# patngnw/NewsRecommendation

Measured on AMD Instinct MI355X. Metric: train impressions/sec @ batch 512, NRMS, higher is better.
Workload: dtype bf16; 1 GPU; NRMS train step (fwd+bwd+Adam), MIND-small shapes: title_len=30, history=50, npratio=4, 300-d word table; per_gpu_batch=512, global_batch=512, vocab_rows=30000, freeze_embedding=False, compact_history=False, dense_batch=False, feed=resident, deterministic=False, optimizer=flat bucket + HIP fused Adam, parallelism=dp1

## Files before the change

include/nrhip.h:

```cpp
#ifndef NRHIP_H
#define NRHIP_H

#include <stddef.h>
#include <stdint.h>

#ifdef __cplusplus
extern "C" {
#endif

#define NR_F32 0
#define NR_BF16 1

#define NR_OK 0
#define NR_ERR_ARG 1
#define NR_ERR_HIP 2

#define NR_SRC_DENSE 0
#define NR_SRC_GATHER 1

typedef void* nr_stream_t;

int nr_version(void);
int nr_last_error(char* buf, size_t n);
int nr_abi_sizes(size_t* out, int n);
// ... 111 lines not shown
                     int dtype, nr_stream_t stream);

typedef struct {
  int M, K, N, dtype;
  int src_kind;
  const void* x;
  int ldx;
  const int32_t* ids;
  int ids_stride;
  const void* w;
  int ldw;
  const float* bias;
  const void* w_t;
  int ldwt;
  size_t dout_ws_bytes;
  int table_rows;
} nr_linear_desc;
size_t nr_linear_workspace_bytes(const nr_linear_desc* d);
int nr_linear_fwd(const nr_linear_desc* d, float* out, int ld_out, nr_stream_t stream);
int nr_linear_bwd(const nr_linear_desc* d, const float* dout, int ld_dout, void* dout_ws, float* dw,
                  float* db, float* dtable, nr_stream_t stream);

int nr_score_ce_fwd(const float* cand, int ld_cand, const float* user, const int64_t* label, float* score,
                    float* loss, float* lossvec, int B, int C, int N, nr_stream_t stream);
int nr_score_ce_bwd(const float* cand, int ld_cand, const float* user, const int64_t* label,
                    const float* score, const float* gloss, const float* gscore, float* dcand, int ld_dcand,
                    float* duser, int B, int C, int N, nr_stream_t stream);
int nr_score_eval(const float* news_vecs, int ld_news, const int32_t* cand_ids, const int32_t* imp_of,
                  const float* user, int ld_user, float* score, int n_cand, int N, nr_stream_t stream);

int nr_assemble_batch(const int32_t* news_combined, int n_rows, int F, const int32_t* hist_idx, const int32_t* pos_idx,
                      const int32_t* neg_idx, const int64_t* label, int B, int H, int K, int32_t* history, int32_t* candidate,
                      int32_t* bad, nr_stream_t stream);

int nr_stack_rows(const int32_t* a, int rows_a, const int32_t* b, int rows_b, int F, const float* mask_b, int32_t* out,
                  int32_t* flags, nr_stream_t stream);

size_t nr_eval_metrics_workspace_bytes(int n_imp);
int nr_eval_metrics(const float* score, const int32_t* label, const int32_t* offsets, int n_imp, int max_cand, double* per_imp,
                    size_t per_imp_bytes, double* sums, nr_stream_t stream);

int nr_adam_step(float* param, float* grad, float* exp_avg, float* exp_avg_sq, size_t n, float lr, float beta1, float beta2, float eps,
                 int step, float grad_scale, int zero_grad, nr_stream_t stream);
#define NR_ADAM_PACK_MAX 4
typedef struct {
  size_t first, count;
  int cols, ld_dst;
// ... 22 lines not shown
```

newsrecommendation_amd/_lib.py:

```python
from __future__ import annotations

import ctypes as C
import os
import subprocess
import threading

NR_F32, NR_BF16 = 0, 1
NR_SRC_DENSE, NR_SRC_GATHER = 0, 1

_HERE = os.path.dirname(os.path.abspath(__file__))
LIB_PATH = os.environ.get("NRHIP_LIB") or os.path.join(_HERE, "libnrhip.so")
CSRC_DIR = os.path.join(_HERE, "csrc")

c_f32p = C.POINTER(C.c_float)
c_i32p = C.POINTER(C.c_int32)
c_i64p = C.POINTER(C.c_int64)


class MhsaDesc(C.Structure):
    _fields_ = [("n", C.c_int), ("L", C.c_int), ("d_model", C.c_int), ("heads", C.c_int), ("d_head", C.c_int),
                ("dtype", C.c_int), ("src_kind", C.c_int), ("x", C.c_void_p), ("ldx", C.c_int), ("ids", C.c_void_p),
                ("p_in", C.c_float), ("seed_in", C.c_uint32), ("p_out", C.c_float), ("seed_out", C.c_uint32),
                ("mask", C.c_void_p), ("w_qkv", C.c_void_p), ("ldw", C.c_int), ("b_qkv", C.c_void_p),
                ("x_rows", C.c_void_p), ("ld_rows", C.c_int), ("row_ws", C.c_void_p), ("row_ws_bytes", C.c_size_t),
# ... 61 lines not shown
    "nr_adam_step": [_vp, _vp, _vp, _vp, C.c_size_t, _f, _f, _f, _f, _i, _f, _i, _vp],
    "nr_adam_step_packed": [_vp, _vp, _vp, _vp, C.c_size_t, _f, _f, _f, _f, _i, _f, _i, _vp, _i, _vp],
    "nr_check_ids": [_vp, _i, _i, _i, _vp, _vp],
    "nr_check_labels": [_vp, _i, _i, _vp, _vp],
    "nr_cast_pad": [_vp, _i, _i, _i, _vp, _i, _i, _i, _vp],
    "nr_cast_pad_batch": [_vp, _i, _i, _vp],
    "nr_pack_conv_w": [_vp, _i, _i, _vp, _i, _i, _vp],
    "nr_unpack_conv_dw": [_vp, _i, _i, _i, _vp, _i, _vp],
    "nr_embed_gather_fwd": [_vp, _i, _i, _vp, _i, _i, _i, _vp, _i, _vp],
    "nr_embed_gather_bwd": [_vp, _i, _vp, _i, _i, _i, _vp, _i, _vp],
    "nr_gather_cast_fwd": [_vp, _i, _vp, _i, _i, _vp, _i, _i, _vp],
    "nr_mhsa_fwd_fused": [C.POINTER(MhsaDesc)],
    "nr_mhsa_compact_rows": [C.POINTER(MhsaDesc)],
    "nr_mhsa_fwd": [C.POINTER(MhsaDesc), _vp, _vp, _vp],
    "nr_mhsa_bwd": [C.POINTER(MhsaDesc), _vp, _vp, _vp, _vp, _i, _vp, _vp, _vp, _vp, _vp],
    "nr_conv1d_k3_fwd": [C.POINTER(ConvDesc), _vp, _vp],
    "nr_conv1d_k3_bwd": [C.POINTER(ConvDesc), _vp, _vp, _vp, _vp],
    "nr_additive_pool_fwd": [C.POINTER(PoolDesc), _vp, _vp, _vp, _i, _vp],
    "nr_additive_pool_bwd": [C.POINTER(PoolDesc), _vp, _vp, _vp, _i, _vp, _i, _vp, _vp, _vp, _vp, _vp, _vp, _vp, _vp],
    "nr_pad_blend_fwd": [_vp, _vp, _vp, _vp, _i, _i, _i, _i, _vp],
    "nr_pad_blend_bwd": [_vp, _vp, _vp, _vp, _i, _i, _i, _i, _vp],
    "nr_linear_fwd": [C.POINTER(LinearDesc), _vp, _i, _vp],
    "nr_linear_bwd": [C.POINTER(LinearDesc), _vp, _i, _vp, _vp, _vp, _vp, _vp],
    "nr_score_ce_fwd": [_vp, _i, _vp, _vp, _vp, _vp, _vp, _i, _i, _i, _vp],
    "nr_score_ce_bwd": [_vp, _i, _vp, _vp, _vp, _vp, _vp, _vp, _i, _vp, _i, _i, _i, _vp],
    "nr_score_eval": [_vp, _i, _vp, _vp, _vp, _i, _vp, _i, _i, _vp],
    "nr_gemm_nt": [_i, _vp, _i, _vp, _i, _vp, _i, _vp, _i, _i, _i, _i, _i, _vp],
    "nr_gemm_tn": [_i, _vp, _i, _vp, _i, _vp, _i, _vp, _i, _i, _i, _vp],
    "nr_dropout_mask": [_vp, _u32, _f, _u32, _vp],
    "nr_prof_enable": [_i],
    "nr_prof_collect": [C.c_char_p, C.c_size_t],
    "nr_prof_filter": [C.c_char_p],
    "nr_debug_nt_trace": [_vp, _i],
}

_lib = None
_lock = threading.Lock()


def build(force: bool = False) -> str:
    if force or not os.path.exists(LIB_PATH):
        subprocess.run(["make", "-C", CSRC_DIR, "-j4"], check=True)
    elif _stale():
        subprocess.run(["make", "-C", CSRC_DIR, "-j4"], check=True)
    return LIB_PATH


# ... 74 lines not shown
```

newsrecommendation_amd/csrc/nr_api.hip:

```cpp
#include <stdarg.h>
#include <stdio.h>
#include <stdlib.h>
#include <string.h>

#include "nr_gemm.h"

int nr_launch_attn(bool bwd, int dtype, const void* qkv, const float* mask, void* y, const void* dy, void* dqkv, int n, int L,
                   int heads, int d_head, const DropCfg& drop, hipStream_t stream, const uint32_t* tmask = nullptr,
                   const float* bias = nullptr, const int32_t* seq_list = nullptr, const int32_t* seq_count = nullptr,
                   const int32_t* needed = nullptr);
bool nr_attn_pad_ok(int dtype, int L, int d_head, const void* p0, const void* p1);
bool nr_attn_rowsub_ok(int dtype, int L, int d_head, int heads);
bool nr_attn_compact_ok(int dtype, int L, int d_head, int heads);
int nr_launch_attn_bwd_compact(const void* qkv, const float* mask, const void* dy, void* dqkv, int n, int L, int heads, int d_head,
                               const DropCfg& drop, hipStream_t stream, const uint32_t* tmask, const float* bias, const int32_t* seq_list,
                               const int32_t* seq_count, const int32_t* pos, void* dump, float* db, const int32_t* nzf);
int nr_launch_attn_gather_fwd(const void* proj_table, const int32_t* ids, const float* mask, void* y, int n, int L, int heads,
                              int d_head, const DropCfg& drop, hipStream_t stream);
int nr_launch_pool_core_fwd(int dtype, const void* x, const void* e, const float* w2, const float* b2, const float* mask,
                            float* alpha, float* out, int ld_out, int n, int L, int N, int q, hipStream_t s,
                            const int32_t* needed = nullptr);
int nr_launch_pool_core_bwd(int dtype, const void* x, const void* e, const float* w2, const float* alpha, const float* g,
                            int ld_g, void* dpre, float* partial, float* dw2, float* db2, int n, int L, int N, int q,
                            hipStream_t s, const int32_t* seq_nz = nullptr);
// ... 224 lines not shown
  memset(&e, 0, sizeof(e));
  e.C = C; e.ldc = ldc; e.out_dtype = out_dtype; e.bias = bias; e.act_tanh = act_tanh;
  e.drop = nr_make_drop(0.f, 0);
  return e;
}

static int mhsa_rows(const nr_mhsa_desc* d, RowSrc* out) {
  RowSrc s = dense_rows(d->x, d->ldx, d->d_model);
  if (d->src_kind == NR_SRC_GATHER) {
    NR_CHECK_ARG(d->ids != nullptr, "mhsa: gather source without ids");
    s.kind = ROWS_GATHER;
    s.ids = d->ids;
  } else {
    NR_CHECK_ARG(d->src_kind == NR_SRC_DENSE, "mhsa: bad src_kind %d", d->src_kind);
  }
  s.drop = nr_make_drop(d->p_in, d->seed_in);
  *out = s;
  return NR_OK;
}

struct MhsaWs {
  size_t live_idx, live_ids, dead_idx, tmask, slab, seq, sort_idx, sort_ids, hist, cursor, pos, sort_k, dump, tn_scratch, tn_floats, total;
};
static MhsaWs mhsa_ws_layout(int n, int L, int table_rows, int N3 = 0, int Kp = 0) {
  const size_t M = (size_t)n * L;
  MhsaWs w;
  w.live_idx = 4; w.live_ids = 4 + M; w.dead_idx = 4 + 2 * M; w.tmask = 4 + 3 * M;
  w.slab = w.tmask + n;
  w.seq = w.slab + n + 4 + M / 32 + 4;
  w.sort_idx = (w.seq + 4 + n + 4 + 3) / 4 * 4;
  w.sort_ids = w.sort_idx + (table_rows > 0 ? (M + 3) / 4 * 4 : 0);
  w.hist = w.sort_ids + (table_rows > 0 ? (M + 3) / 4 * 4 : 0);
  w.cursor = w.hist + (table_rows > 0 ? (size_t)table_rows + 8 : 0);
  w.pos = (w.cursor + (table_rows > 0 ? (size_t)table_rows + 8 : 0) + 3) / 4 * 4;
  w.sort_k = w.pos + (table_rows > 0 ? (M + 3) / 4 * 4 : 0);
  w.dump = w.sort_k + (table_rows > 0 ? (M + 3) / 4 * 4 : 0);
  w.tn_scratch = (w.dump + (table_rows > 0 ? 1024 : 0) + 3) / 4 * 4;
  w.tn_floats = (table_rows > 0 && N3 >= 8 && Kp >= 8 && M % 32 == 0) ? nr_gemm_tn_scratch_floats((int)M, N3, Kp) : 0;
  w.total = w.tn_scratch + w.tn_floats;
  return w;
}
static MhsaWs mhsa_ws_of(const nr_mhsa_desc* d) {
  const bool gather = d->src_kind == NR_SRC_GATHER;
  const int ch = dtype_ok(d->dtype) ? nr_chunk(d->dtype) : 4;
  return mhsa_ws_layout(d->n, d->L, gather ? d->table_rows : 0, gather && d->dtype == NR_BF16 ? 3 * d->heads * d->d_head : 0,
                        gather && d->dtype == NR_BF16 ? round_up(d->d_model, ch) : 0);
}
static size_t conv_ws_elems(int n, int T) { return (size_t)n + 4 + ((size_t)n * T) / 32 + 12; }
int nr_pool_partial_rows(int n);
static size_t pool_ws_used(int n, int q) { return ((size_t)nr_pool_partial_rows(n) * (q + 1) + 3) / 4 * 4; }
static size_t pool_ws_ints(int n, int L, int q) { return (pool_ws_used(n, q) + (size_t)n + 8 + ((size_t)n * L) / 32 + 4 + 3) / 4 * 4; }
static size_t pool_tn_floats(int n, int L, int q, int N, int dtype) {
  const size_t M = (size_t)n * L;
  return (dtype == NR_BF16 && q >= 8 && N >= 8 && M % 32 == 0 && M > 0) ? nr_gemm_tn_scratch_floats((int)M, q, N) : 0;
}
static size_t pool_ws_elems(int n, int L, int q, int N = 0, int dtype = NR_F32) { return pool_ws_ints(n, L, q) + pool_tn_floats(n, L, q, N, dtype); }

static bool pool_has_flags(const nr_pool_desc* d) {
  const int M = d->n * d->L;
  return !nr_opt(NR_OPT_NO_SLABS) && d->dtype == NR_BF16 && M % 32 == 0 && d->L <= 32 && nr_gemm_tn_slabs_ok(d->q, d->N, M, d->q, d->N);
}

static bool conv_slab_shape(const nr_conv_desc* d) {
  const int M = d->n * d->T;
  return !nr_opt(NR_OPT_NO_SLABS) && d->dtype == NR_BF16 && d->x_rows != nullptr && M % 32 == 0 && d->T <= 32 && d->N % 8 == 0 &&
         nr_gemm_tn_slabs_ok(d->N, d->ld_rows, M, d->N, 3 * d->Dp);
}

static bool mhsa_compact_rows(const nr_mhsa_desc* d) {
// ... 424 lines not shown
        if (d->table_rows > 0 && !nr_opt(NR_OPT_NO_SCATTER_SORT)) {
          if ((rc = nr_launch_sort_rows_by_id(d->row_ws, ep.row_idx, ep.row_ids, M, d->table_rows, d->row_ws + W.hist,
                                              d->row_ws + W.sort_idx, d->row_ws + W.sort_ids, s)))
            return rc;
          ep.row_idx = d->row_ws + W.sort_idx; ep.row_ids = d->row_ws + W.sort_ids;
        }
      }
      rc = nr_launch_gemm_nt(d->dtype, G, w_qkv_t, ldwt, M, d->d_model, 3 * N, EPI_SCATTER, ep, s);
    } else {
      NR_CHECK_ARG(dx != nullptr && dtable == nullptr, "mhsa_bwd: dense source takes dx, not dtable");
      NR_CHECK_ARG(d->p_in == 0.f, "mhsa_bwd: input dropout on a dense source is not supported");
      NR_CHECK_ARG(d->d_model % 4 == 0, "mhsa_bwd: d_model=%d must be a multiple of 4", d->d_model);
      EpiArgs ep = store_epi(dx, d->ldx, d->dtype, nullptr, 0);
      rc = nr_launch_gemm_nt(d->dtype, G, w_qkv_t, ldwt, M, d->d_model, 3 * N, EPI_STORE, ep, s);
    }
  }
  if (rc) return rc;
  if (ph_dw) {
    if (slab_ws != nullptr) {
      if ((rc = nr_launch_gemm_tn_slabs(dqkv, 3 * N, d->x_rows, d->ld_rows, dw_qkv, d->d_model, db_qkv, M, 3 * N, Kp, 3 * N, d->d_model,
                                        slab_ws + d->n + 4, slab_ws + d->n, s, 0,
                                        W.tn_floats ? reinterpret_cast<float*>(d->row_ws + W.tn_scratch) : nullptr, W.tn_floats)))
        return rc;
    } else if ((rc = nr_launch_gemm_tn(d->dtype, dqkv, 3 * N, Xs, dw_qkv, d->d_model, db_qkv, M, 3 * N, Kp, 3 * N, d->d_model, s))) {
      return rc;
    }
  }
  if (fork) {
    const int rj = side_join(s);
    if (rc == NR_OK) rc = rj;
  }
  const int rd = det.end();
  return rc ? rc : rd;
}

static int conv_rows(const nr_conv_desc* d, RowSrc* out) {
  NR_CHECK_ARG(d != nullptr, "conv1d: null descriptor");
  NR_CHECK_ARG(dtype_ok(d->dtype), "conv1d: bad dtype %d", d->dtype);
  const int ch = nr_chunk(d->dtype);
  NR_CHECK_ARG(d->n >= 0 && d->T >= 1 && d->D >= 1 && d->N >= 1 && d->Dp >= d->D && d->Dp % ch == 0,
               "conv1d: bad shape n=%d T=%d D=%d Dp=%d N=%d", d->n, d->T, d->D, d->Dp, d->N);
  NR_CHECK_ARG(d->N % ch == 0, "conv1d: N=%d must be a multiple of %d", d->N, ch);
  NR_CHECK_ARG(d->n == 0 || (d->table && d->ids && d->w_pack && d->bias && d->ids_stride >= 1), "conv1d: null operand");
  NR_CHECK_ARG((uint64_t)d->n * d->T * (uint64_t)d->D < 0xffffffffull, "conv1d: problem too large for 32-bit element counters");
  RowSrc s = dense_rows(d->table, d->Dp, d->D);
  s.kind = ROWS_IM2COL3;
  s.ids = d->ids; s.ids_stride = d->ids_stride; s.Tlen = d->T;
// ... 120 lines not shown
  const int32_t* zero_flags = ws != nullptr ? ws : d->seq_needed;
  if (ws != nullptr && dx != nullptr && w1_t != nullptr && !det.on() && nr_pool_fused_bwd_ok(d->dtype, d->n, d->L, d->N, d->q, ldw1t) && ld_g % 4 == 0 &&
      ((((uintptr_t)d->x) | ((uintptr_t)e) | ((uintptr_t)w1_t) | ((uintptr_t)dpre) | ((uintptr_t)dx) | ((uintptr_t)g)) & 15) == 0 && d->N % 8 == 0) {
    int rows = 0;
    if ((rc = nr_launch_pool_fused_bwd(d->x, d->N, e, d->q, alpha, g, ld_g, d->w2, w1_t, ldw1t, dpre, d->q, dx, d->N, partial,
                                       nr_pool_partial_rows(d->n), ws, d->n, d->L, d->N, d->q, s, &rows, d->dx_far_unwritten)))
      return rc;
    if ((rc = nr_launch_colsum_split(partial, rows, d->q + 1, d->q + 1, dw2, d->q, db2, s))) return rc;
    if ((rc = nr_launch_live_slabs(ws, d->n, d->L, s))) return rc;
    return nr_launch_gemm_tn_slabs(dpre, d->q, d->x, d->N, dw1, d->N, db1, M, d->q, d->N, d->q, d->N, ws + d->n + 4, ws + d->n, s, 0,
                                   tn_floats ? tn_scratch : nullptr, tn_floats);
  }
  if ((rc = nr_launch_pool_core_bwd(d->dtype, d->x, e, d->w2, alpha, g, ld_g, dpre, partial, dw2, db2, d->n, d->L, d->N, d->q, s, zero_flags)))
    return rc;
  RowSrc X = dense_rows(d->x, d->N, d->N);
  const bool fork = dx != nullptr && side_enabled() && M >= 65536 && !det.on();
  hipStream_t s2 = s;
  if (fork && (rc = side_fork(s, &s2))) return rc;
  if (ws != nullptr) {
    if ((rc = nr_launch_live_slabs(ws, d->n, d->L, s))) return rc;
    if ((rc = nr_launch_gemm_tn_slabs(dpre, d->q, d->x, d->N, dw1, d->N, db1, M, d->q, d->N, d->q, d->N, ws + d->n + 4, ws + d->n, s, 0,
                                      tn_floats ? tn_scratch : nullptr, tn_floats)))
      return rc;
  } else if ((rc = nr_launch_gemm_tn(d->dtype, dpre, d->q, X, dw1, d->N, db1, M, d->q, d->N, d->q, d->N, s))) {
    return rc;
  }
  if (dx != nullptr) {
    NR_CHECK_ARG(w1_t != nullptr && ldw1t >= d->q, "additive_pool_bwd: w1_t [N, >=q] needed for dx");
    RowSrc P = dense_rows(dpre, d->q, d->q);
    EpiArgs ep = store_epi(dx, d->N, d->dtype, nullptr, 0);
    ep.rowscale = alpha; ep.G = g; ep.ldg = ld_g; ep.L = d->L;
    ep.seq_nz = zero_flags;
    rc = nr_launch_gemm_nt(d->dtype, P, w1_t, ldw1t, M, d->N, d->q, EPI_POOLBWD, ep, s2);
  }
  if (fork) {
    const int rj = side_join(s);
    if (rc == NR_OK) rc = rj;
  }
  return rc;
}

static int linear_rows(const nr_linear_desc* d, RowSrc* out) {
  NR_CHECK_ARG(d != nullptr, "linear: null descriptor");
  NR_CHECK_ARG(dtype_ok(d->dtype), "linear: bad dtype %d", d->dtype);
  const int ch = nr_chunk(d->dtype);
  NR_CHECK_ARG(d->M >= 0 && d->K >= 1 && d->N >= 1, "linear: bad shape M=%d K=%d N=%d", d->M, d->K, d->N);
  NR_CHECK_ARG(d->ldx >= round_up(d->K, ch) && d->ldw >= round_up(d->K, ch), "linear: ldx=%d / ldw=%d must cover K=%d rounded up to %d",
// ... 59 lines not shown
```

newsrecommendation_amd/csrc/nr_gemm.h:

```cpp
#pragma once
#include "nr_common.h"

enum { ROWS_DENSE = 0, ROWS_GATHER = 1, ROWS_IM2COL3 = 2 };

struct RowSrc {
  const void* base;
  const int32_t* ids;
  int ld;
  int ids_stride;
  int kind;
  int Tlen;
  int Dtrue;
  DropCfg drop;
  int gap;
};

enum {
  EPI_STORE = 0,
  EPI_POOLBWD = 1,
  EPI_SCATTER = 2,
  EPI_STORE_TANH = 3,
};

struct EpiArgs {
// ... 41 lines not shown
                          bool zeroed = false);
int nr_launch_seq_list(const int32_t* title_nz, const uint32_t* tmask, int n, int L, int32_t* out, hipStream_t stream, int reach = -1,
                       bool zeroed = false);
int nr_launch_zero_tail_rows(void* buf, int ld, const int32_t* count, int Mmax, hipStream_t stream, int32_t* za = nullptr, int na = 0,
                             int32_t* zb = nullptr, int nb = 0);
int nr_launch_gemm_tn_slabs(const void* dC, int ldc, const void* X, int ldx, float* dW, int ldw, float* db, int M, int N, int K,
                            int Nstore, int Kstore, const int32_t* slab_list, const int32_t* slab_count, hipStream_t stream, int xgap = 0,
                            float* scratch = nullptr, size_t scratch_floats = 0);
size_t nr_gemm_tn_scratch_floats(int M, int N, int K);
bool nr_gemm_tn_slabs_ok(int ldc, int ldx, int M, int N, int K);
int nr_pool_fused_fwd_ok(int dtype, int n, int L, int N, int q, int ldw1);
int nr_launch_pool_fused_fwd(const void* x, int ldx, const void* w1, int ldw1, const float* b1, const float* w2, const float* b2,
                             const float* mask, void* e, int lde, float* alpha, float* out, int ld_out, int n, int L, int N, int q,
                             const int32_t* needed, hipStream_t stream);
int nr_launch_gemm_tn_counted(const void* dC, int ldc, const void* X, int ldx, float* dW, int ldw, int Mmax, int N, int K, int Nstore,
                              int Kstore, const int32_t* row_count, hipStream_t stream, float* scratch = nullptr, size_t scratch_floats = 0);
int nr_pool_fused_bwd_ok(int dtype, int n, int L, int N, int q, int ldw1t);
int nr_launch_pool_fused_bwd(const void* x, int ldx, const void* e, int lde, const float* alpha, const float* g, int ldg, const float* w2,
                             const void* w1t, int ldw1t, void* dpre, int ldp, void* dx, int lddx, float* partial, int partial_rows,
                             const int32_t* nz, int n, int L, int N, int q, hipStream_t stream, int* grid_out, int dx_far_unwritten = 0);
int nr_launch_gather_live_rows(int dtype, const RowSrc& A, void* out, int ldo, int Mmax, int K, const int32_t* count, const int32_t* rows,
                               const int32_t* ids, hipStream_t stream, int32_t* hist = nullptr, int V = 0);
int nr_launch_gemm_tn(int dtype, const void* dC, int ldc, const RowSrc& A, float* dW, int ldw, float* db,
                      int M, int N, int K, int Nstore, int Kstore, hipStream_t stream);
```

newsrecommendation_amd/csrc/nr_gemm.hip:

```cpp
#include <stdlib.h>

#include "nr_gemm.h"

namespace {

constexpr int BM = 128, BN = 128, BK = 32, NTHR = 256;
constexpr int SC = BN + 4;

template <typename T> struct TileCfg {
  static constexpr int CH = 16 / (int)sizeof(T);
  static constexpr int SK = BK + CH;
  static constexpr int CPR = BK / CH;
  static constexpr int NCH = BM * CPR / NTHR;
  static constexpr int RPC = BM / CH;
  static constexpr size_t STAGE_BYTES = (size_t)2 * 2 * BM * SK * sizeof(T);
};
constexpr size_t EPI_BYTES = (size_t)64 * SC * sizeof(float);

template <typename T> constexpr size_t smem_bytes() {
  return TileCfg<T>::STAGE_BYTES > EPI_BYTES ? TileCfg<T>::STAGE_BYTES : EPI_BYTES;
}

union Chunk {
  uint4 u;
// ... 3542 lines not shown
  hipLaunchKernelGGL(live_slabs_kernel, dim3(1), dim3(1024), in_lds ? (size_t)((n + 15) / 16) * 16 : 0, stream, ws, n, L, nslab, ws + n,
                     list, in_lds);
  NR_CHECK_LAUNCH();
  return NR_OK;
}

int nr_launch_gemm_tn_slabs(const void* dC, int ldc, const void* X, int ldx, float* dW, int ldw, float* db, int M, int N, int K,
                            int Nstore, int Kstore, const int32_t* slab_list, const int32_t* slab_count, hipStream_t stream, int xgap,
                            float* scratch, size_t scratch_floats) {
  NR_CHECK_ARG(tn3::eligible(ldc, ldx, M, N, K), "gemm_tn_slabs: shape not eligible");
  NrProfScope ps(stream, "gemm_tn3_live[bf16,Mmax=%d,N=%d,K=%d,gap=%d]", M, N, K, xgap);
  return tn3::launch(dC, ldc, X, ldx, dW, ldw, db, M, N, K, Nstore, Kstore, stream, slab_list, slab_count, xgap, scratch, scratch_floats);
}
size_t nr_gemm_tn_scratch_floats(int M, int N, int K) { return tn3::scratch_floats(M, N, K); }
bool nr_gemm_tn_slabs_ok(int ldc, int ldx, int M, int N, int K) { return tn3::eligible(ldc, ldx, M, N, K); }
int nr_launch_gemm_tn_counted(const void* dC, int ldc, const void* X, int ldx, float* dW, int ldw, int Mmax, int N, int K, int Nstore,
                              int Kstore, const int32_t* row_count, hipStream_t stream, float* scratch, size_t scratch_floats) {
  NR_CHECK_ARG(tn3::eligible(ldc, ldx, Mmax, N, K) && row_count != nullptr, "gemm_tn_counted: shape not eligible");
  NrProfScope ps(stream, "gemm_tn3_rows[bf16,Mmax=%d,N=%d,K=%d,gap=0]", Mmax, N, K);
  return tn3::launch(dC, ldc, X, ldx, dW, ldw, nullptr, Mmax, N, K, Nstore, Kstore, stream, nullptr, row_count, 0, scratch, scratch_floats);
}

int nr_launch_gemm_tn(int dtype, const void* dC, int ldc, const RowSrc& A, float* dW, int ldw, float* db, int M, int N,
                      int K, int Nstore, int Kstore, hipStream_t stream) {
  const int ch = nr_chunk(dtype);
  NR_CHECK_ARG(M > 0 && N > 0 && K > 0, "gemm_tn: empty problem M=%d N=%d K=%d", M, N, K);
  NR_CHECK_ARG(N % ch == 0 && K % ch == 0 && ldc % ch == 0 && A.ld % ch == 0, "gemm_tn: N=%d K=%d ldc=%d lda=%d must be multiples of %d",
               N, K, ldc, A.ld, ch);
  NR_CHECK_ARG(((uintptr_t)A.base & 15) == 0 && ((uintptr_t)dC & 15) == 0, "gemm_tn: operands must be 16-byte aligned");
  const bool tn_v1 = nr_opt(NR_OPT_TN_V1) != 0;
  if (!tn_v1 && dtype == NR_BF16 && A.kind == ROWS_DENSE && A.drop.thresh == 0) {
    if (tn3::eligible(ldc, A.ld, M, N, K)) {
      NrProfScope ps(stream, "gemm_tn3[bf16,M=%d,N=%d,K=%d,gap=%d]", M, N, K, A.gap);
      return tn3::launch(dC, ldc, A.base, A.ld, dW, ldw, db, M, N, K, Nstore, Kstore, stream, nullptr, nullptr, A.gap);
    }
    if (A.gap == 0) {
      NrProfScope ps(stream, "gemm_tn2[bf16,M=%d,N=%d,K=%d]", M, N, K);
      return tn2::launch(dC, ldc, A.base, A.ld, dW, ldw, db, M, N, K, Nstore, Kstore, stream);
    }
  }
  NrProfScope ps(stream, "gemm_tn[%s,rows=%d,M=%d,N=%d,K=%d]", dtype == NR_BF16 ? "bf16" : "f32", A.kind, M, N, K);
  return dtype == NR_BF16 ? launch_tn_d<bf16_t>(dC, ldc, A, dW, ldw, db, M, N, K, Nstore, Kstore, stream)
                          : launch_tn_d<float>(dC, ldc, A, dW, ldw, db, M, N, K, Nstore, Kstore, stream);
}
```

newsrecommendation_amd/csrc/nr_pool.hip:

```cpp
#include "nr_common.h"

namespace {

template <typename T> struct ChunkOf { static constexpr int CH = 16 / (int)sizeof(T); };
template <typename T> __device__ __forceinline__ void load_chunk_f(const T* p, float (&f)[ChunkOf<T>::CH]);
template <> __device__ __forceinline__ void load_chunk_f<float>(const float* p, float (&f)[4]) {
  const f32x4 v = *reinterpret_cast<const f32x4*>(p);
  f[0] = v[0]; f[1] = v[1]; f[2] = v[2]; f[3] = v[3];
}
template <> __device__ __forceinline__ void load_chunk_f<bf16_t>(const bf16_t* p, float (&f)[8]) {
  const bf16x8 v = *reinterpret_cast<const bf16x8*>(p);
#pragma unroll
  for (int e = 0; e < 8; ++e) f[e] = (float)v[e];
}
template <typename T> __device__ __forceinline__ void store_chunk_f(T* p, const float (&f)[ChunkOf<T>::CH]);
template <> __device__ __forceinline__ void store_chunk_f<float>(float* p, const float (&f)[4]) {
  *reinterpret_cast<f32x4*>(p) = (f32x4){f[0], f[1], f[2], f[3]};
}
template <> __device__ __forceinline__ void store_chunk_f<bf16_t>(bf16_t* p, const float (&f)[8]) {
  bf16x8 v;
#pragma unroll
  for (int e = 0; e < 8; ++e) v[e] = (bf16_t)f[e];
  *reinterpret_cast<bf16x8*>(p) = v;
}
// ... 291 lines not shown
  const float* u = user + (size_t)b * N;
  float my = -INFINITY;
  for (int j0 = 0; j0 < C; j0 += 8) {
    float p[8] = {0.f, 0.f, 0.f, 0.f, 0.f, 0.f, 0.f, 0.f};
    for (int c = lane; c < N; c += 64) {
      const float uc = u[c];
#pragma unroll
      for (int t = 0; t < 8; ++t)
        if (j0 + t < C) p[t] = fmaf(cand[((size_t)b * C + j0 + t) * ld_cand + c], uc, p[t]);
    }
#pragma unroll
    for (int t = 0; t < 8; ++t) {
      const float q = wave_sum(p[t]);
      if (lane == j0 + t) my = q;
    }
  }
  if (lane < C) score[(size_t)b * C + lane] = my;
  const float m = wave_max(my);
  const float ex = lane < C ? expf(my - m) : 0.f;
  const float lse = m + logf(wave_sum(ex));
  const int lab = (int)label[b];
  const float sl = __shfl(my, lab, 64);
  if (lane == 0) lossvec[b] = lse - sl;
}

__global__ __launch_bounds__(256) void mean_kernel(const float* __restrict__ v, int n, float* __restrict__ out) {
  __shared__ float red[256];
  float s = 0.f;
  for (int i = threadIdx.x; i < n; i += 256) s += v[i];
  red[threadIdx.x] = s;
  __syncthreads();
  for (int o = 128; o > 0; o >>= 1) {
    if (threadIdx.x < o) red[threadIdx.x] += red[threadIdx.x + o];
    __syncthreads();
  }
  if (threadIdx.x == 0) out[0] = red[0] / (float)n;
}

__global__ __launch_bounds__(256) void score_ce_bwd_kernel(const float* __restrict__ cand, int ld_cand,
                                                           const float* __restrict__ user,
                                                           const int64_t* __restrict__ label,
                                                           const float* __restrict__ score,
                                                           const float* __restrict__ gloss,
                                                           const float* __restrict__ gscore, float inv_b,
                                                           float* __restrict__ dcand, int ld_dcand,
                                                           float* __restrict__ duser, int C, int N) {
// ... 413 lines not shown
  int det_rc = NR_OK;
  const int det = (mask != nullptr && dpad != nullptr) ? nr_det_open(s, dpad, (size_t)N, nullptr, 0, false, true, &det_rc) : 0;
  if (det_rc) return det_rc;
  NrProfScope ps(s, "pad_blend_bwd[n=%d,L=%d,N=%d]", n, L, N);
  if (N % 4 == 0 && N / 4 <= 256 && (((uintptr_t)dout | (uintptr_t)dx) & 15) == 0) {
    const int rl_n = 256 / (N / 4), rpb4 = 64;
    const size_t smem = (size_t)rl_n * N * sizeof(float);
    if (dtype == NR_BF16)
      hipLaunchKernelGGL(blend_bwd4_kernel<bf16_t>, dim3((rows + rpb4 - 1) / rpb4), dim3(256), smem, s, (const bf16_t*)dout, mask, dx, dpad, rows, N, rpb4);
    else
      hipLaunchKernelGGL(blend_bwd4_kernel<float>, dim3((rows + rpb4 - 1) / rpb4), dim3(256), smem, s, (const float*)dout, mask, dx, dpad, rows, N, rpb4);
    NR_CHECK_LAUNCH();
    return nr_det_close(det);
  }
  if (dtype == NR_BF16)
    hipLaunchKernelGGL(blend_bwd_kernel<bf16_t>, dim3((rows + rpb - 1) / rpb), dim3(256), 0, s, (const bf16_t*)dout, mask, dx, dpad, rows, N, rpb);
  else
    hipLaunchKernelGGL(blend_bwd_kernel<float>, dim3((rows + rpb - 1) / rpb), dim3(256), 0, s, (const float*)dout, mask, dx, dpad, rows, N, rpb);
  NR_CHECK_LAUNCH();
  return nr_det_close(det);
}

int nr_score_ce_fwd(const float* cand, int ld_cand, const float* user, const int64_t* label, float* score, float* loss,
                    float* lossvec, int B, int C, int N, nr_stream_t stream) {
  NR_CHECK_ARG(cand && user && label && score && loss && lossvec, "score_ce_fwd: null pointer");
  NR_CHECK_ARG(B > 0 && C >= 1 && C <= 64 && N > 0, "score_ce_fwd: B=%d C=%d (1..64) N=%d", B, C, N);
  NR_DEVICE_GUARD(stream, score);
  hipStream_t s = (hipStream_t)stream;
  NrProfScope ps(s, "score_ce_fwd[B=%d,C=%d,N=%d]", B, C, N);
  hipLaunchKernelGGL(score_ce_fwd_kernel, dim3(B), dim3(64), 0, s, cand, ld_cand, user, label, score, lossvec, C, N);
  hipLaunchKernelGGL(mean_kernel, dim3(1), dim3(256), 0, s, lossvec, B, loss);
  NR_CHECK_LAUNCH();
  return NR_OK;
}

int nr_score_ce_bwd(const float* cand, int ld_cand, const float* user, const int64_t* label, const float* score,
                    const float* gloss, const float* gscore, float* dcand, int ld_dcand, float* duser, int B, int C, int N,
                    nr_stream_t stream) {
  NR_CHECK_ARG(cand && user && label && score && dcand && duser, "score_ce_bwd: null pointer");
  NR_CHECK_ARG(B > 0 && C >= 1 && C <= 64 && N > 0, "score_ce_bwd: B=%d C=%d (1..64) N=%d", B, C, N);
  NR_DEVICE_GUARD(stream, dcand);
  NrProfScope ps((hipStream_t)stream, "score_ce_bwd[B=%d,C=%d,N=%d]", B, C, N);
  hipLaunchKernelGGL(score_ce_bwd_kernel, dim3(B), dim3(256), 0, (hipStream_t)stream, cand, ld_cand, user, label, score, gloss, gscore, 1.0f / (float)B, dcand, ld_dcand, duser, C, N);
  NR_CHECK_LAUNCH();
  return NR_OK;
}

int nr_score_eval(const float* news_vecs, int ld_news, const int32_t* cand_ids, const int32_t* imp_of, const float* user,
                  int ld_user, float* score, int n_cand, int N, nr_stream_t stream) {
  NR_CHECK_ARG(news_vecs && cand_ids && imp_of && user && score, "score_eval: null pointer");
  NR_DEVICE_GUARD(stream, score);
  if (n_cand == 0) return NR_OK;
  hipLaunchKernelGGL(score_eval_kernel, dim3((n_cand + 3) / 4), dim3(256), 0, (hipStream_t)stream, news_vecs, ld_news, cand_ids, imp_of, user, ld_user, score, n_cand, N);
  NR_CHECK_LAUNCH();
// ... 15 lines not shown
```

newsrecommendation_amd/ops.py:

```python
from __future__ import annotations

import ctypes as C
import os
import weakref
from typing import Optional

import torch
from torch.autograd import Function

from . import _lib
from ._lib import NR_BF16, NR_F32, NR_SRC_DENSE, NR_SRC_GATHER, check, ptr

_DTYPES = {"fp32": NR_F32, "f32": NR_F32, "float32": NR_F32, "bf16": NR_BF16, "bfloat16": NR_BF16}


def dtype_code(name) -> int:
    if isinstance(name, int):
        return name
    try:
        return _DTYPES[str(name).lower()]
    except KeyError:
        raise ValueError(f"compute dtype must be one of {sorted(_DTYPES)}, got {name!r}")


# ... 339 lines not shown
            dw, db = flat[:3 * N * d_model].view(3 * N, d_model), flat[3 * N * d_model:]
        need_x = ctx.needs_input_grad[0]
        dx = dtable = w_t = None
        row_ws = getattr(ctx, "row_ws", None)
        ws_ready = row_ws is not None
        d = _lib.MhsaDesc(n=n, L=L, d_model=d_model, heads=heads, d_head=d_head, dtype=code,
                          src_kind=NR_SRC_GATHER if gather else NR_SRC_DENSE, x=ptr(src), ldx=ldx, ids=ptr(ids),
                          p_in=cfg["p_in"], seed_in=cfg["seed_in"], p_out=cfg["p_out"], seed_out=cfg["seed_out"],
                          mask=ptr(mask_c), w_qkv=ptr(w_p), ldw=w_p.shape[1], b_qkv=ptr(b_p),
                          x_rows=ptr(x_rows), ld_rows=x_rows.shape[1] if x_rows is not None else 0,
                          table_rows=cfg["table_shape"][0] if gather else 0, seq_nz=seq_nz, row_ws_ready=int(ws_ready),
                          dy_far_unwritten=int(dy_lazy),
                          seq_needed=ptr(cfg.get("needed")))
        if need_x:
            w_t = pack(wcat, code, transpose=True)
            if gather:
                dtable = cfg.get("table_grad")
                if dtable is None:
                    dtable = torch.zeros(cfg["table_shape"], dtype=torch.float32, device=dev)
                if row_ws is None:
                    row_ws = _ws(_lib.lib().nr_mhsa_workspace_bytes(C.byref(d)), dev)
            else:
                dx = torch.empty(n, L, ldx, dtype=torch_dtype(code), device=dev)
        d.row_ws, d.row_ws_bytes = ptr(row_ws), (row_ws.numel() * 4 if row_ws is not None else 0)
        def run(phase):
            d.bwd_phase = phase
            check(_lib.lib().nr_mhsa_bwd(C.byref(d), ptr(qkv), ptr(dy), ptr(dqkv), ptr(w_t), w_t.shape[1] if w_t is not None else 0,
                                         ptr(dw), ptr(db), ptr(dx), ptr(dtable), _stream()), "nr_mhsa_bwd")
        ready = cfg.get("table_grad_ready") if (gather and cfg.get("table_grad") is not None and _det_scratch is None) else None
        if ready is not None:
            run(1)
            ready()
            run(2)
        else:
            run(0)
        gx = (None if cfg.get("table_grad") is not None else dtable) if gather else dx
        if bucket is not None:
            return (gx, None, None, None, None, None, None, None, None, None)
        return (gx, dw[:N], db[:N], dw[N:2 * N], db[N:2 * N], dw[2 * N:], db[2 * N:], None, None, None)


USE_PROJECTED_TABLE = True


def _mhsa_projected(table, params, flat, ids, mask, heads, code, p_out):
    wq, bq, wk, bk, wv, bv = params
# ... 224 lines not shown
        n, L, N = ctx.dims
        dout = dout.contiguous()
        if dout.dtype != torch_dtype(ctx.code):
            dout = dout.to(torch_dtype(ctx.code))
        dx = ctx.dx_out.view(n, L, N) if ctx.dx_out is not None else torch.empty(n, L, N, dtype=torch.float32, device=dout.device)
        direct = ctx.pad_target is not None and mask_c is not None
        dpad = ctx.pad_target if direct else (torch.zeros(N, dtype=torch.float32, device=dout.device) if mask_c is not None else None)
        check(_lib.lib().nr_pad_blend_bwd(ptr(dout), ptr(mask_c), ptr(dx), ptr(dpad), n, L, N, ctx.code, _stream()), "nr_pad_blend_bwd")
        if direct:
            return dx, None, None, None
        return dx, None, (dpad.view(ctx.pad_shape) if dpad is not None and ctx.pad_shape is not None else None), None


def pad_blend(x, mask, pad, code: int):
    return BlendFunction.apply(x, mask, pad, code)


def to_compute(x, code: int):
    if x.dtype == torch_dtype(code) and code == NR_F32:
        return x
    return BlendFunction.apply(x, None, None, code)


class ScoreCEFunction(Function):

    @staticmethod
    def forward(ctx, cand, user, label):
        _need_gpu(cand, user, label)
        B, Cn, N = cand.shape
        cand, user = cand.contiguous().float(), user.contiguous().float()
        label = label.contiguous().to(torch.int64)
        score = torch.empty(B, Cn, dtype=torch.float32, device=cand.device)
        loss = torch.empty((), dtype=torch.float32, device=cand.device)
        lossvec = torch.empty(B, dtype=torch.float32, device=cand.device)
        check(_lib.lib().nr_score_ce_fwd(ptr(cand), N, ptr(user), ptr(label), ptr(score), ptr(loss), ptr(lossvec), B, Cn, N,
                                         _stream()), "nr_score_ce_fwd")
        ctx.save_for_backward(cand, user, label, score)
        ctx.dcand_out = _take_grad_out(cand)
        ctx.set_materialize_grads(False)
        return loss, score

    @staticmethod
    def backward(ctx, gloss, gscore):
        _enter_backward()
        cand, user, label, score = ctx.saved_tensors
        B, Cn, N = cand.shape
        gl = gloss.contiguous().float() if gloss is not None else None
        gs = gscore.contiguous().float() if gscore is not None else None
        dcand = ctx.dcand_out.view_as(cand) if ctx.dcand_out is not None else torch.empty_like(cand)
        duser = torch.empty_like(user)
        check(_lib.lib().nr_score_ce_bwd(ptr(cand), N, ptr(user), ptr(label), ptr(score), ptr(gl), ptr(gs), ptr(dcand), N,
                                         ptr(duser), B, Cn, N, _stream()), "nr_score_ce_bwd")
        return dcand, duser, None


def score_ce(cand, user, label):
    if CHECK_INDICES:
        check_labels(label.contiguous().to(torch.int64), cand.shape[1])
    return ScoreCEFunction.apply(cand, user, label)
# ... 235 lines not shown
```

Measured before the change: 174,200 impressions/s.

## Fuse score-CE loss mean into scoring kernel and give dense gemm_tn scratch

Replaces the per-sample scoring kernel (one wave per sample) plus a separate mean kernel with a single kernel that handles four samples per block using vectorized loads. The last block, found through an atomic counter, reduces the per-sample losses into the mean loss. This removes one launch and the tiny serial mean kernel, at the cost of a persistent counter tensor and a threadfence. The mhsa and pool backward paths also now pass a scratch workspace to the dense bf16 gemm_tn (tn3) so it can use its split/scratch path, and a workspace is allocated for dense bf16 MHSA backward.

```diff
diff --git a/include/nrhip.h b/include/nrhip.h
--- a/include/nrhip.h
+++ b/include/nrhip.h
@@ -157,7 +157,7 @@
                   float* db, float* dtable, nr_stream_t stream);
 
 int nr_score_ce_fwd(const float* cand, int ld_cand, const float* user, const int64_t* label, float* score,
-                    float* loss, float* lossvec, int B, int C, int N, nr_stream_t stream);
+                    float* loss, float* lossvec, unsigned int* counter, int B, int C, int N, nr_stream_t stream);
 int nr_score_ce_bwd(const float* cand, int ld_cand, const float* user, const int64_t* label,
                     const float* score, const float* gloss, const float* gscore, float* dcand, int ld_dcand,
                     float* duser, int B, int C, int N, nr_stream_t stream);
diff --git a/newsrecommendation_amd/_lib.py b/newsrecommendation_amd/_lib.py
--- a/newsrecommendation_amd/_lib.py
+++ b/newsrecommendation_amd/_lib.py
@@ -107,7 +107,7 @@
     "nr_pad_blend_bwd": [_vp, _vp, _vp, _vp, _i, _i, _i, _i, _vp],
     "nr_linear_fwd": [C.POINTER(LinearDesc), _vp, _i, _vp],
     "nr_linear_bwd": [C.POINTER(LinearDesc), _vp, _i, _vp, _vp, _vp, _vp, _vp],
-    "nr_score_ce_fwd": [_vp, _i, _vp, _vp, _vp, _vp, _vp, _i, _i, _i, _vp],
+    "nr_score_ce_fwd": [_vp, _i, _vp, _vp, _vp, _vp, _vp, _vp, _i, _i, _i, _vp],
     "nr_score_ce_bwd": [_vp, _i, _vp, _vp, _vp, _vp, _vp, _vp, _i, _vp, _i, _i, _i, _vp],
     "nr_score_eval": [_vp, _i, _vp, _vp, _vp, _i, _vp, _i, _i, _vp],
     "nr_gemm_nt": [_i, _vp, _i, _vp, _i, _vp, _i, _vp, _i, _i, _i, _i, _i, _vp],
diff --git a/newsrecommendation_amd/csrc/nr_api.hip b/newsrecommendation_amd/csrc/nr_api.hip
--- a/newsrecommendation_amd/csrc/nr_api.hip
+++ b/newsrecommendation_amd/csrc/nr_api.hip
@@ -270,7 +270,7 @@
 struct MhsaWs {
   size_t live_idx, live_ids, dead_idx, tmask, slab, seq, sort_idx, sort_ids, hist, cursor, pos, sort_k, dump, tn_scratch, tn_floats, total;
 };
-static MhsaWs mhsa_ws_layout(int n, int L, int table_rows, int N3 = 0, int Kp = 0) {
+static MhsaWs mhsa_ws_layout(int n, int L, int table_rows, int N3 = 0, int Kp = 0, bool dense = false) {
   const size_t M = (size_t)n * L;
   MhsaWs w;
   w.live_idx = 4; w.live_ids = 4 + M; w.dead_idx = 4 + 2 * M; w.tmask = 4 + 3 * M;
@@ -284,15 +284,15 @@
   w.sort_k = w.pos + (table_rows > 0 ? (M + 3) / 4 * 4 : 0);
   w.dump = w.sort_k + (table_rows > 0 ? (M + 3) / 4 * 4 : 0);
   w.tn_scratch = (w.dump + (table_rows > 0 ? 1024 : 0) + 3) / 4 * 4;
-  w.tn_floats = (table_rows > 0 && N3 >= 8 && Kp >= 8 && M % 32 == 0) ? nr_gemm_tn_scratch_floats((int)M, N3, Kp) : 0;
+  w.tn_floats = ((table_rows > 0 || dense) && N3 >= 8 && Kp >= 8 && M % 32 == 0) ? nr_gemm_tn_scratch_floats((int)M, N3, Kp) : 0;
   w.total = w.tn_scratch + w.tn_floats;
   return w;
 }
 static MhsaWs mhsa_ws_of(const nr_mhsa_desc* d) {
   const bool gather = d->src_kind == NR_SRC_GATHER;
   const int ch = dtype_ok(d->dtype) ? nr_chunk(d->dtype) : 4;
-  return mhsa_ws_layout(d->n, d->L, gather ? d->table_rows : 0, gather && d->dtype == NR_BF16 ? 3 * d->heads * d->d_head : 0,
-                        gather && d->dtype == NR_BF16 ? round_up(d->d_model, ch) : 0);
+  return mhsa_ws_layout(d->n, d->L, gather ? d->table_rows : 0, d->dtype == NR_BF16 ? 3 * d->heads * d->d_head : 0,
+                        d->dtype == NR_BF16 ? round_up(d->d_model, ch) : 0, !gather);
 }
 static size_t conv_ws_elems(int n, int T) { return (size_t)n + 4 + ((size_t)n * T) / 32 + 12; }
 int nr_pool_partial_rows(int n);
@@ -763,7 +763,9 @@
                                         slab_ws + d->n + 4, slab_ws + d->n, s, 0,
                                         W.tn_floats ? reinterpret_cast<float*>(d->row_ws + W.tn_scratch) : nullptr, W.tn_floats)))
         return rc;
-    } else if ((rc = nr_launch_gemm_tn(d->dtype, dqkv, 3 * N, Xs, dw_qkv, d->d_model, db_qkv, M, 3 * N, Kp, 3 * N, d->d_model, s))) {
+    } else if ((rc = nr_launch_gemm_tn(d->dtype, dqkv, 3 * N, Xs, dw_qkv, d->d_model, db_qkv, M, 3 * N, Kp, 3 * N, d->d_model, s,
+                                       d->row_ws != nullptr && W.tn_floats ? reinterpret_cast<float*>(d->row_ws + W.tn_scratch) : nullptr,
+                                       d->row_ws != nullptr ? W.tn_floats : 0))) {
       return rc;
     }
   }
@@ -930,7 +932,8 @@
     if ((rc = nr_launch_gemm_tn_slabs(dpre, d->q, d->x, d->N, dw1, d->N, db1, M, d->q, d->N, d->q, d->N, ws + d->n + 4, ws + d->n, s, 0,
                                       tn_floats ? tn_scratch : nullptr, tn_floats)))
       return rc;
-  } else if ((rc = nr_launch_gemm_tn(d->dtype, dpre, d->q, X, dw1, d->N, db1, M, d->q, d->N, d->q, d->N, s))) {
+  } else if ((rc = nr_launch_gemm_tn(d->dtype, dpre, d->q, X, dw1, d->N, db1, M, d->q, d->N, d->q, d->N, s, tn_floats ? tn_scratch : nullptr,
+                                     tn_floats))) {
     return rc;
   }
   if (dx != nullptr) {
diff --git a/newsrecommendation_amd/csrc/nr_gemm.h b/newsrecommendation_amd/csrc/nr_gemm.h
--- a/newsrecommendation_amd/csrc/nr_gemm.h
+++ b/newsrecommendation_amd/csrc/nr_gemm.h
@@ -87,4 +87,4 @@
 int nr_launch_gather_live_rows(int dtype, const RowSrc& A, void* out, int ldo, int Mmax, int K, const int32_t* count, const int32_t* rows,
                                const int32_t* ids, hipStream_t stream, int32_t* hist = nullptr, int V = 0);
 int nr_launch_gemm_tn(int dtype, const void* dC, int ldc, const RowSrc& A, float* dW, int ldw, float* db,
-                      int M, int N, int K, int Nstore, int Kstore, hipStream_t stream);
+                      int M, int N, int K, int Nstore, int Kstore, hipStream_t stream, float* scratch = nullptr, size_t scratch_floats = 0);
diff --git a/newsrecommendation_amd/csrc/nr_gemm.hip b/newsrecommendation_amd/csrc/nr_gemm.hip
--- a/newsrecommendation_amd/csrc/nr_gemm.hip
+++ b/newsrecommendation_amd/csrc/nr_gemm.hip
@@ -3588,7 +3588,7 @@
 }
 
 int nr_launch_gemm_tn(int dtype, const void* dC, int ldc, const RowSrc& A, float* dW, int ldw, float* db, int M, int N,
-                      int K, int Nstore, int Kstore, hipStream_t stream) {
+                      int K, int Nstore, int Kstore, hipStream_t stream, float* scratch, size_t scratch_floats) {
   const int ch = nr_chunk(dtype);
   NR_CHECK_ARG(M > 0 && N > 0 && K > 0, "gemm_tn: empty problem M=%d N=%d K=%d", M, N, K);
   NR_CHECK_ARG(N % ch == 0 && K % ch == 0 && ldc % ch == 0 && A.ld % ch == 0, "gemm_tn: N=%d K=%d ldc=%d lda=%d must be multiples of %d",
@@ -3598,7 +3598,7 @@
   if (!tn_v1 && dtype == NR_BF16 && A.kind == ROWS_DENSE && A.drop.thresh == 0) {
     if (tn3::eligible(ldc, A.ld, M, N, K)) {
       NrProfScope ps(stream, "gemm_tn3[bf16,M=%d,N=%d,K=%d,gap=%d]", M, N, K, A.gap);
-      return tn3::launch(dC, ldc, A.base, A.ld, dW, ldw, db, M, N, K, Nstore, Kstore, stream, nullptr, nullptr, A.gap);
+      return tn3::launch(dC, ldc, A.base, A.ld, dW, ldw, db, M, N, K, Nstore, Kstore, stream, nullptr, nullptr, A.gap, scratch, scratch_floats);
     }
     if (A.gap == 0) {
       NrProfScope ps(stream, "gemm_tn2[bf16,M=%d,N=%d,K=%d]", M, N, K);
diff --git a/newsrecommendation_amd/csrc/nr_pool.hip b/newsrecommendation_amd/csrc/nr_pool.hip
--- a/newsrecommendation_amd/csrc/nr_pool.hip
+++ b/newsrecommendation_amd/csrc/nr_pool.hip
@@ -337,6 +337,59 @@
   const int lab = (int)label[b];
   const float sl = __shfl(my, lab, 64);
   if (lane == 0) lossvec[b] = lse - sl;
+}
+
+__global__ __launch_bounds__(256) void score_ce_fwd4_kernel(const float* __restrict__ cand, int ld_cand,
+                                                            const float* __restrict__ user,
+                                                            const int64_t* __restrict__ label, float* __restrict__ score,
+                                                            float* lossvec, float* __restrict__ loss,
+                                                            unsigned int* __restrict__ counter, int B, int C, int N) {
+  __shared__ float red[256];
+  __shared__ int is_last;
+  const int tid = threadIdx.x, lane = tid & 63, b = blockIdx.x * 4 + (tid >> 6);
+  if (b < B) {
+    const float* u = user + (size_t)b * N;
+    float my = -INFINITY;
+    for (int j0 = 0; j0 < C; j0 += 8) {
+      float p[8] = {0.f, 0.f, 0.f, 0.f, 0.f, 0.f, 0.f, 0.f};
+      for (int c = 4 * lane; c < N; c += 256) {
+        const f32x4 uc = *reinterpret_cast<const f32x4*>(u + c);
+        f32x4 cv[8];
+#pragma unroll
+        for (int t = 0; t < 8; ++t)
+          if (j0 + t < C) cv[t] = *reinterpret_cast<const f32x4*>(cand + ((size_t)b * C + j0 + t) * ld_cand + c);
+#pragma unroll
+        for (int t = 0; t < 8; ++t)
+          if (j0 + t < C) p[t] = fmaf(cv[t][0], uc[0], fmaf(cv[t][1], uc[1], fmaf(cv[t][2], uc[2], fmaf(cv[t][3], uc[3], p[t]))));
+      }
+#pragma unroll
+      for (int t = 0; t < 8; ++t) {
+        const float q = wave_sum(p[t]);
+        if (lane == j0 + t) my = q;
+      }
+    }
+    if (lane < C) score[(size_t)b * C + lane] = my;
+    const float m = wave_max(my);
+    const float ex = lane < C ? expf(my - m) : 0.f;
+    const float lse = m + logf(wave_sum(ex));
+    const float sl = __shfl(my, (int)label[b], 64);
+    if (lane == 0) lossvec[b] = lse - sl;
+  }
+  __threadfence();
+  __syncthreads();
+  if (tid == 0) is_last = atomicInc(counter, gridDim.x - 1) == gridDim.x - 1;
+  __syncthreads();
+  if (!is_last) return;
+  __threadfence();
+  float s = 0.f;
+  for (int i = tid; i < B; i += 256) s += lossvec[i];
+  red[tid] = s;
+  __syncthreads();
+  for (int o = 128; o > 0; o >>= 1) {
+    if (tid < o) red[tid] += red[tid + o];
+    __syncthreads();
+  }
+  if (tid == 0) loss[0] = red[0] / (float)B;
 }
 
 __global__ __launch_bounds__(256) void mean_kernel(const float* __restrict__ v, int n, float* __restrict__ out) {
@@ -796,14 +849,19 @@
 }
 
 int nr_score_ce_fwd(const float* cand, int ld_cand, const float* user, const int64_t* label, float* score, float* loss,
-                    float* lossvec, int B, int C, int N, nr_stream_t stream) {
+                    float* lossvec, unsigned int* counter, int B, int C, int N, nr_stream_t stream) {
   NR_CHECK_ARG(cand && user && label && score && loss && lossvec, "score_ce_fwd: null pointer");
   NR_CHECK_ARG(B > 0 && C >= 1 && C <= 64 && N > 0, "score_ce_fwd: B=%d C=%d (1..64) N=%d", B, C, N);
   NR_DEVICE_GUARD(stream, score);
   hipStream_t s = (hipStream_t)stream;
   NrProfScope ps(s, "score_ce_fwd[B=%d,C=%d,N=%d]", B, C, N);
-  hipLaunchKernelGGL(score_ce_fwd_kernel, dim3(B), dim3(64), 0, s, cand, ld_cand, user, label, score, lossvec, C, N);
-  hipLaunchKernelGGL(mean_kernel, dim3(1), dim3(256), 0, s, lossvec, B, loss);
+  if (counter != nullptr && N % 4 == 0 && ld_cand % 4 == 0 && ((((uintptr_t)cand) | ((uintptr_t)user)) & 15) == 0) {
+    hipLaunchKernelGGL(score_ce_fwd4_kernel, dim3((B + 3) / 4), dim3(256), 0, s, cand, ld_cand, user, label, score, lossvec, loss, counter,
+                       B, C, N);
+  } else {
+    hipLaunchKernelGGL(score_ce_fwd_kernel, dim3(B), dim3(64), 0, s, cand, ld_cand, user, label, score, lossvec, C, N);
+    hipLaunchKernelGGL(mean_kernel, dim3(1), dim3(256), 0, s, lossvec, B, loss);
+  }
   NR_CHECK_LAUNCH();
   return NR_OK;
 }
diff --git a/newsrecommendation_amd/ops.py b/newsrecommendation_amd/ops.py
--- a/newsrecommendation_amd/ops.py
+++ b/newsrecommendation_amd/ops.py
@@ -385,6 +385,8 @@
                     row_ws = _ws(_lib.lib().nr_mhsa_workspace_bytes(C.byref(d)), dev)
             else:
                 dx = torch.empty(n, L, ldx, dtype=torch_dtype(code), device=dev)
+        if not gather and code == _lib.NR_BF16:
+            row_ws = _ws(_lib.lib().nr_mhsa_workspace_bytes(C.byref(d)), dev)
         d.row_ws, d.row_ws_bytes = ptr(row_ws), (row_ws.numel() * 4 if row_ws is not None else 0)
         def run(phase):
             d.bwd_phase = phase
@@ -655,6 +657,17 @@
     return BlendFunction.apply(x, None, None, code)
 
 
+_done_counters = {}
+
+
+def _done_counter(device) -> torch.Tensor:
+    key = (device, _stream())
+    t = _done_counters.get(key)
+    if t is None:
+        t = _done_counters[key] = torch.zeros(1, dtype=torch.int32, device=device)
+    return t
+
+
 class ScoreCEFunction(Function):
 
     @staticmethod
@@ -666,8 +679,8 @@
         score = torch.empty(B, Cn, dtype=torch.float32, device=cand.device)
         loss = torch.empty((), dtype=torch.float32, device=cand.device)
         lossvec = torch.empty(B, dtype=torch.float32, device=cand.device)
-        check(_lib.lib().nr_score_ce_fwd(ptr(cand), N, ptr(user), ptr(label), ptr(score), ptr(loss), ptr(lossvec), B, Cn, N,
-                                         _stream()), "nr_score_ce_fwd")
+        check(_lib.lib().nr_score_ce_fwd(ptr(cand), N, ptr(user), ptr(label), ptr(score), ptr(loss), ptr(lossvec),
+                                         ptr(_done_counter(cand.device)), B, Cn, N, _stream()), "nr_score_ce_fwd")
         ctx.save_for_backward(cand, user, label, score)
         ctx.dcand_out = _take_grad_out(cand)
         ctx.set_materialize_grads(False)
```

Result: no change. 175,000 impressions/s (median of 4 runs) (+0.5%).
